# spectralcode/OCTproZ

Measured on AMD Instinct MI355X. Metric: A-scans/s, higher is better.
Workload: dtype f32

## Files before the change

octproz_amd/csrc/kernels.h:

```cpp
#pragma once
#ifndef __HIPCC_RTC__
#include <hip/hip_runtime.h>
#endif
#include <stdint.h>

#include "fft_regs.h"

namespace oct {

enum { IN_U8 = 0, IN_U16 = 1, IN_U32 = 2, IN_F32 = 3, IN_P12U = 4, IN_P12S = 5, IN_I16 = 6 };
enum { RS_NONE = 0, RS_LINEAR = 1, RS_CUBIC = 2, RS_LANCZOS = 3 };

struct FusedArgs {
	const void* raw;
	float* out;
	f2* spectrum;
	const float4* lut;
	const f2* twiddle;
	const f2* meanLine;
	unsigned numLines;
	unsigned linesInBuffer;
	unsigned ascansPerBscan;
	int bitshift;
	int rollingW;
	int rollExact;
	int flip;
	int subtractMean;
	float sA, sB;
	const float* lanczosW;
	const float* bgTerm;
	const float4* cubicW;
	float* dispBscan;
	float* dispEnFace;
	unsigned dispBscanRow0;
	unsigned dispEnFaceBin;
	unsigned dispEnFaceLast;
	const uint32_t* sinEnt;
	unsigned sinM, sinTotal, sinBlk;
};

#ifndef OCT_CW11
#define OCT_CW11 8
#endif
#ifndef OCT_PRIO_GATHER
#define OCT_PRIO_GATHER 3
#endif
#ifndef OCT_PRIO_FFT
#define OCT_PRIO_FFT 2
#endif
#ifndef OCT_PRIO_EPILOGUE
#define OCT_PRIO_EPILOGUE 1
#endif
#ifndef OCT_PRIO_STAGING
#define OCT_PRIO_STAGING 0
// ... 11 lines not shown
template <> struct GatherCfg<8> { static constexpr int GROUP = 4; static constexpr bool AHEAD = false; };
#if defined(__HIP_DEVICE_COMPILE__) && !defined(__gfx950__) && !defined(__gfx942__) && !defined(__gfx90a__)
#error "kernels.h is written for gfx9 (MI355X: gfx950)"
#endif
OCT_DEV void prologue_wait() {
	__builtin_amdgcn_s_waitcnt(0x0F70);
}
template <int LOG2N> struct Cfg;
template <> struct Cfg<8>  { static constexpr bool PLANAR = false; static constexpr int WAVES_ROLL = 0; static constexpr int WAVES = 8,  MINW = 4; static constexpr bool LDS_LUT = true; static constexpr bool PRIO = true; static constexpr bool MEAN_REGS = true; static constexpr int WAVES_CW = 8; };
template <> struct Cfg<9>  { static constexpr bool PLANAR = false; static constexpr int WAVES_ROLL = 0; static constexpr int WAVES = 8,  MINW = 4; static constexpr bool LDS_LUT = true; static constexpr bool PRIO = true; static constexpr bool MEAN_REGS = true; static constexpr int WAVES_CW = 8; };
template <> struct Cfg<10> { static constexpr bool PLANAR = false; static constexpr int WAVES_ROLL = 12; static constexpr int WAVES = 16, MINW = 4; static constexpr bool LDS_LUT = true; static constexpr bool PRIO = true; static constexpr bool MEAN_REGS = true; static constexpr int WAVES_CW = 8; };
template <> struct Cfg<11> { static constexpr bool PLANAR = true; static constexpr int WAVES_ROLL = OCT_CW11 ? 5 : 6; static constexpr int WAVES = 12, MINW = 3; static constexpr bool LDS_LUT = true; static constexpr bool PRIO = true; static constexpr bool MEAN_REGS = false; static constexpr int WAVES_CW = OCT_CW11; };
template <> struct Cfg<12> { static constexpr bool PLANAR = true; static constexpr int WAVES_ROLL = 3; static constexpr int WAVES = 6,  MINW = 2; static constexpr bool LDS_LUT = false; static constexpr bool PRIO = true; static constexpr bool MEAN_REGS = false; static constexpr int WAVES_CW = 0; };
template <int LOG2N, int RS, bool ROLL = false> struct KCfg {
	static constexpr bool CW = RS == RS_CUBIC && Cfg<LOG2N>::LDS_LUT && Cfg<LOG2N>::WAVES_CW > 0;
	static constexpr bool MEAN_REGS = Cfg<LOG2N>::MEAN_REGS || (CW && LOG2N == 11);
	static constexpr bool REGTAB = CW && LOG2N <= 10;
	static constexpr bool REGLIN = !CW && LOG2N <= 10 && (RS == RS_LINEAR || RS == RS_NONE) && !ROLL;
	static constexpr bool LZ_LDS = RS == RS_LANCZOS && LOG2N <= 10 && Cfg<LOG2N>::LDS_LUT;
	static constexpr int WAVES_PLAIN = REGLIN ? (LOG2N <= 9 ? Cfg<LOG2N>::WAVES : RS == RS_NONE ? 12 : 8) : CW ? Cfg<LOG2N>::WAVES_CW : (LZ_LDS && LOG2N == 10) ? 8 : Cfg<LOG2N>::WAVES;
	static constexpr int WAVES = (ROLL && Cfg<LOG2N>::WAVES_ROLL > 0 && Cfg<LOG2N>::WAVES_ROLL < WAVES_PLAIN) ? Cfg<LOG2N>::WAVES_ROLL : WAVES_PLAIN;
	static constexpr int MINW = ((REGTAB || REGLIN) && LOG2N <= 9) ? 4 : (REGLIN && RS == RS_NONE) ? 3 : (REGTAB || REGLIN || (LZ_LDS && LOG2N == 10)) ? 2 : (ROLL && Cfg<LOG2N>::WAVES_ROLL > 0) ? (WAVES + 3) / 4 : (CW && LOG2N == 11) ? (WAVES + 3) / 4 : Cfg<LOG2N>::MINW;
};

#ifndef OCT_LANCZOS_AHEAD
#define OCT_LANCZOS_AHEAD 2
#endif
#ifndef OCT_PADK
#define OCT_PADK 1
#endif
constexpr int ROW_OFF = 12;
// ... 416 lines not shown
		f32x4* p3 = p2 + 8 * 16;
		for (int i = tid; i < 8 * 16; i += threads) {
			const int c = i >> 4, k = i & 15;
			const f2 w0 = c ? g[(2 * c - 1) * 16 + k] : f2{1.0f, 0.0f}, w1 = g[(2 * c) * 16 + k];
			p2[i] = f32x4{w0.x, w0.y, w1.x, w1.y};
		}
		for (int i = tid; i < 6 * 64; i += threads) {
			const int c = i >> 6, l = i & 63, i0 = 2 * c, i1 = 2 * c + 1;
			const f2 w0 = g[T2 + (i0 % 3) * 256 + l + 64 * (i0 / 3)], w1 = g[T2 + (i1 % 3) * 256 + l + 64 * (i1 / 3)];
			p3[i] = f32x4{w0.x, w0.y, w1.x, w1.y};
		}
	} else {
		for (int i = tid; i < twiddle_count<LOG2N>(); i += threads) tw[i] = g[i];
	}
}
template <int LOG2N, int RS> constexpr int mean_lds_bytes() { return KCfg<LOG2N, RS>::MEAN_REGS ? 0 : (1 << LOG2N) * 4; }
template <int LOG2N, int RS, bool ROLL = false> constexpr int lut_lds_bytes() { return (!Cfg<LOG2N>::LDS_LUT || KCfg<LOG2N, RS>::REGTAB || KCfg<LOG2N, RS, ROLL>::REGLIN) ? 0 : (1 << LOG2N) * (KCfg<LOG2N, RS>::CW ? 24 : 12) + (KCfg<LOG2N, RS>::LZ_LDS ? (1 << LOG2N) * 64 : 0); }
template <int LOG2N, int RS, bool ROLL> constexpr int block_lds_bytes() {
	return tw_lds_bytes<LOG2N>() + mean_lds_bytes<LOG2N, RS>() + lut_lds_bytes<LOG2N, RS, ROLL>() + KCfg<LOG2N, RS, ROLL>::WAVES * wave_lds_bytes<(1 << LOG2N), ROLL>();
}

OCT_DEV unsigned flipped_row(const FusedArgs& a, unsigned line) {
	const unsigned b = line / a.ascansPerBscan, as = line - b * a.ascansPerBscan;
	return ((b & 1u) == 0u && (b + 2u) * a.ascansPerBscan <= a.linesInBuffer) ? b * a.ascansPerBscan + (a.ascansPerBscan - 1u - as) : line;
}
template <bool> OCT_DEV void ef_flush(const FusedArgs& a, float acc, unsigned first, unsigned stride, int lane, unsigned count) {
	if ((unsigned)lane < count) {
		const unsigned line = first + (unsigned)lane * stride;
		a.dispEnFace[a.dispEnFaceLast - (a.flip ? flipped_row(a, line) : line)] = acc;
	}
}

enum { MODE_ROLL = 1, MODE_SPECTRUM = 2, MODE_LOG = 4, MODE_BG = 8, MODE_DISP = 16, MODE_SINUS = 32 };
template <int MODE, int LOG2N, int RS> constexpr int sinus_lds_bytes() {
// ... 64 lines not shown
		const uint32_t b0 = e0.y, b1 = e0.z;
		*f0 = __builtin_bit_cast(float, b0);
		*f1 = __builtin_bit_cast(float, b1);
		const unsigned r0 = out_row();
		const bool p = sT > 0u && *f0 >= 0.0f;
		*st0 = p && r0 + 1u != lines;
		*st1 = p && *f1 >= 0.0f && r0 + 2u != lines;
		*raw = sBA0 + (e0.x & 0xffffu) + 1u == lines;
	}
};

template <int LOG2N, int INTYPE, int RS, int MODE>
__global__ __launch_bounds__((KCfg<LOG2N, RS, (MODE & 1) != 0>::WAVES) * 64, (KCfg<LOG2N, RS, (MODE & 1) != 0>::MINW)) void oct_fused_kernel(const FusedArgs a) {
	constexpr int N = 1 << LOG2N, P = N / 64;
	constexpr int WAVES = KCfg<LOG2N, RS, (MODE & MODE_ROLL) != 0>::WAVES, THREADS = WAVES * 64;
	constexpr bool LDS_LUT = Cfg<LOG2N>::LDS_LUT, CW = KCfg<LOG2N, RS>::CW, MEAN_REGS = KCfg<LOG2N, RS>::MEAN_REGS, REGTAB = KCfg<LOG2N, RS>::REGTAB;
	constexpr bool REGLIN = KCfg<LOG2N, RS, (MODE & 1) != 0>::REGLIN && RS != RS_LANCZOS;
	constexpr int RL = LastRadix<LOG2N>::value, NBL = P / RL;
	constexpr bool ROLL = (MODE & MODE_ROLL) != 0, SPECTRUM = (MODE & MODE_SPECTRUM) != 0, LOGSCALE = (MODE & MODE_LOG) != 0;
	constexpr bool SINUS = (MODE & MODE_SINUS) != 0;
	static_assert(!(SINUS && (SPECTRUM || (MODE & MODE_DISP) != 0 || RS == RS_LANCZOS)), "sinusoidal correction in the store: image output of the raw-row variants, display frames by the extraction kernel");
	typedef Chunk<INTYPE, N> CH;
	constexpr int SPL = CH::SPL, CB = CH::BYTES, NL = N / (64 * SPL);
	static_assert(!(RS == RS_LANCZOS && INTYPE != IN_F32 && INTYPE != IN_U16), "Lanczos: prepared float buffer or raw uint16 rows");
	static_assert(!(RS == RS_LANCZOS && (MODE & MODE_ROLL) != 0), "Lanczos taps cross line borders: the rolling average of the neighbour rows comes prepared");
	static_assert(!(ROLL && INTYPE != IN_U16), "in-kernel rolling average: uint16 rows only (everything else comes prepared)");
	static_assert(N / (64 * SPL) >= 1, "a row holds at least one chunk per lane");
	extern __shared__ __attribute__((aligned(16))) char smem[];
	f2* tw = reinterpret_cast<f2*>(smem);
	f2* meanL = reinterpret_cast<f2*>(smem + tw_lds_bytes<LOG2N>());
	float* rhoL = reinterpret_cast<float*>(smem + tw_lds_bytes<LOG2N>() + mean_lds_bytes<LOG2N, RS>());
	f32x4* cwL = reinterpret_cast<f32x4*>(rhoL);
	f2* wphL = reinterpret_cast<f2*>(smem + tw_lds_bytes<LOG2N>() + mean_lds_bytes<LOG2N, RS>() + N * (CW ? 16 : 4));
	constexpr bool LZ_LDS = KCfg<LOG2N, RS>::LZ_LDS;
	f32x4* lzL = reinterpret_cast<f32x4*>(smem + tw_lds_bytes<LOG2N>() + mean_lds_bytes<LOG2N, RS>() + N * 12);
	const int tid = threadIdx.x, lane = tid & 63;
	const int wave = __builtin_amdgcn_readfirstlane(tid >> 6);
	char* wbase = smem + tw_lds_bytes<LOG2N>() + mean_lds_bytes<LOG2N, RS>() + lut_lds_bytes<LOG2N, RS, ROLL>() + wave * wave_lds_bytes<N, ROLL>();
	float* row = reinterpret_cast<float*>(wbase);
	f2* xbuf = reinterpret_cast<f2*>(wbase);

	const float* termL = reinterpret_cast<const float*>(smem + block_lds_bytes<LOG2N, RS, ROLL>());
	constexpr bool SINUS_PREV_LDS = sinus_prev_lds<MODE, LOG2N, RS>();
	float* sPrevL = reinterpret_cast<float*>(smem + block_lds_bytes<LOG2N, RS, ROLL>() + bg_lds_bytes<MODE, N>()) + wave * (N / 2);
	float sPrevR[SINUS && !SINUS_PREV_LDS ? P / 2 : 1];
	if constexpr (SINUS && !SINUS_PREV_LDS) {
#pragma unroll
		for (int i = 0; i < P / 2; i++) sPrevR[i] = 0.0f;
	}
	if constexpr ((MODE & MODE_BG) != 0) fill_bg_term(reinterpret_cast<float*>(smem + block_lds_bytes<LOG2N, RS, ROLL>()), a.bgTerm, N / 2, tid, THREADS);
	fill_twiddles<LOG2N>(tw, a.twiddle, tid, THREADS);
	if constexpr (LZ_LDS) {
		const f32x4* g = reinterpret_cast<const f32x4*>(a.lanczosW);
		for (int u = tid; u < N * 4; u += THREADS) lzL[u] = g[((u & 63) + 64 * (u >> 8)) * 4 + ((u >> 6) & 3)];
	}
	if constexpr (!MEAN_REGS)
		for (int i = tid; i < N / 2; i += THREADS) meanL[i] = a.subtractMean ? a.meanLine[i] : f2{0.0f, 0.0f};
	if constexpr (LDS_LUT && !REGTAB && !REGLIN) {
		for (int i = tid; i < N; i += THREADS) {
			const float4 t = a.lut[i];
			wphL[CW ? (((i >> 7) << 6) + (i & 63)) * 2 + ((i >> 6) & 1) : i] = f2{t.y * t.z, t.y * t.w};
			if constexpr (CW) {
				const float4 w = a.cubicW[i];
				cwL[i] = f32x4{w.x, w.y, w.z, w.w};
			} else {
				rhoL[i] = t.x;
			}
		}
	}
	__syncthreads();

	const unsigned wavesTotal = gridDim.x * (unsigned)WAVES;
#ifndef OCT_DISP_BLOCK
#define OCT_DISP_BLOCK 16
#endif
	constexpr unsigned BLK = (MODE & MODE_DISP) != 0 ? (unsigned)OCT_DISP_BLOCK : 1u;
	static_assert(BLK >= 1 && BLK <= 64, "a block's en-face values live in the lanes of one register");
	const unsigned blockStride = wavesTotal * BLK;
	const unsigned blk = blockIdx.x;
	unsigned line = (blk * (unsigned)WAVES + (unsigned)wave) * BLK;
	unsigned inBlock = 0;
	SinusWalk sw;
	if constexpr (SINUS) line = sw.begin(a, blk * (unsigned)WAVES + (unsigned)wave, wavesTotal);
	auto next_line = [&](unsigned ln, unsigned pos) -> unsigned {
		if (BLK > 1u && pos + 1u < BLK) return ln + 1u;
// ... 28 lines not shown
	};
	f2 mreg[MEAN_REGS && !SPECTRUM ? P / 2 : 1];
	if constexpr (MEAN_REGS && !SPECTRUM) {
#pragma unroll
		for (int u = 0; u < RL / 2; u++)
#pragma unroll
			for (int m = 0; m < NBL; m++)
				mreg[m + u * NBL] = a.subtractMean ? a.meanLine[fft_bin<LOG2N>(lane, m, u)] : f2{0.0f, 0.0f};
	}
	float* rowl = row + ROW_OFF + lane;
	uint32_t tapA[CW ? P : 1];
	typedef __attribute__((address_space(3))) const float lds_cfloat;
	const uint32_t tapBase = __builtin_amdgcn_readfirstlane(
	    (uint32_t)(uintptr_t)(__attribute__((address_space(3))) float*)(row + ROW_OFF - 1));

	if constexpr (CW) {
#pragma unroll
		for (int q = 0; q < P; q++) tapA[q] = tapBase + 4u * (uint32_t)(int)a.lut[lane + 64 * q].x;
	}
	f32x4 cwR[REGTAB ? P : 1];
	f2 wphR[REGTAB || REGLIN ? P : 1];
	float fracR[REGLIN && RS == RS_LINEAR ? P : 1];
	uint32_t tapL[REGLIN && RS == RS_LINEAR ? P : 1];
	if constexpr (REGLIN) {
#pragma unroll
		for (int q = 0; q < P; q++) {
			const float4 t = a.lut[lane + 64 * q];
			wphR[q] = f2{t.y * t.z, t.y * t.w};
			if constexpr (RS == RS_LINEAR) {
				fracR[q] = __builtin_amdgcn_fractf(t.x);
				tapL[q] = tapBase + 4u * (uint32_t)(int)t.x + 4u;
			}
		}
	}
	constexpr bool TW3 = (REGTAB || REGLIN) && LOG2N == 10 && !ROLL && INTYPE != IN_F32;
	constexpr bool TW2 = (REGTAB || REGLIN) && LOG2N == 10 && !ROLL;
	f32x4 tw2R[TW2 ? (TW3 ? 14 : 8) : 1];
	if constexpr (REGTAB) {
#pragma unroll
		for (int q = 0; q < P; q++) {
			const float4 t = a.lut[lane + 64 * q];
			wphR[q] = f2{t.y * t.z, t.y * t.w};
			const float4 w = a.cubicW[lane + 64 * q];
			cwR[q] = f32x4{w.x, w.y, w.z, w.w};
		}
	}
	if constexpr (TW2) {
#pragma unroll
		for (int c = 0; c < 8; c++) tw2R[c] = reinterpret_cast<const f32x4*>(tw)[c * 16 + (lane & 15)];
	}
	if constexpr (TW3) {
#pragma unroll
		for (int c = 0; c < 6; c++) tw2R[8 + c] = reinterpret_cast<const f32x4*>(tw)[8 * 16 + c * 64 + lane];
	}
	float rollCnt[ROLL ? 8 : 1], rollRc[ROLL ? 8 : 1];
	if constexpr (ROLL) {
#pragma unroll
		for (int e = 0; e < 8; e++) {
			const int j = 4 * lane + (e < 4 ? 0 : 256 * (NL - 1)) + (e & 3);
			const int lo = max(0, j - a.rollingW + 1), hi = min(N - 1, j + a.rollingW);
			rollCnt[e] = (float)(hi - lo + 1);
			rollRc[e] = __fdiv_rn(1.0f, rollCnt[e]);
		}
	}
	constexpr bool DISP = (MODE & MODE_DISP) != 0;
	static_assert(!(DISP && SPECTRUM), "display frames are copies of the image");
	const unsigned efIdx = DISP ? __builtin_amdgcn_readfirstlane(a.dispEnFaceBin >> 6) : 0u, efLane = DISP ? __builtin_amdgcn_readfirstlane(a.dispEnFaceBin & 63u) : 0u;
	float efAcc = 0.0f;
	unsigned efCount = 0, efFirst = line;
	prologue_wait();
	while (line < lineEnd) {
		if constexpr (SINUS) sw.load_ahead();
		if constexpr (RS != RS_LANCZOS) {
			bool staged = false;
			if constexpr (ROLL) {
				const int W = a.rollingW;
				{
					staged = true;
					uint32_t* pfx = reinterpret_cast<uint32_t*>(row + N + 2 * ROW_OFF);
					uint32_t base = 0;
#pragma unroll
					for (int i = 0; i < NL; i++) {
						const uint4 x = chunk_to_uint(pre[i], 0, shift);
						const uint32_t tot = x.x + x.y + x.z + x.w;
						const uint32_t incl = wave_inclusive_scan(tot);
						const uint32_t p3 = base + incl, p2 = p3 - x.w, p1 = p2 - x.z, p0 = p1 - x.y;
						*reinterpret_cast<uint4*>(&pfx[ROLL_PAD + 4 * lane + 256 * i]) = uint4{p0, p1, p2, p3};
						base += (uint32_t)__builtin_amdgcn_readlane((int)incl, 63);
					}
					static_assert(ROLL_PAD == 256, "pad writes: four entries per lane");
					*reinterpret_cast<uint4*>(&pfx[4 * lane]) = uint4{0u, 0u, 0u, 0u};
					*reinterpret_cast<uint4*>(&pfx[ROLL_PAD + N + 4 * lane]) = uint4{base, base, base, base};
					wave_sync_lds();
					const uint32_t* hiP = pfx + ROLL_PAD + 4 * lane + W;
					const uint32_t* loP = pfx + ROLL_PAD + 4 * lane - W;
					const float cntIn = (float)(2 * W), rcIn = __fdiv_rn(1.0f, cntIn);
					const bool quad = (W & 3) == 0;
					const bool fast = a.rollExact == 2;
					uint32_t wsAll[NL][4];
					if (quad) {
						uint4 h4[NL], l4[NL];
#pragma unroll
						for (int i = 0; i < NL; i++) { h4[i] = *reinterpret_cast<const uint4*>(hiP + 256 * i); l4[i] = *reinterpret_cast<const uint4*>(loP + 256 * i); }
#pragma unroll
						for (int i = 0; i < NL; i++) { wsAll[i][0] = h4[i].x - l4[i].x; wsAll[i][1] = h4[i].y - l4[i].y; wsAll[i][2] = h4[i].z - l4[i].z; wsAll[i][3] = h4[i].w - l4[i].w; }
					} else {
#pragma unroll
						for (int i = 0; i < NL; i++)
#pragma unroll
							for (int c = 0; c < 4; c++) wsAll[i][c] = hiP[256 * i + c] - loP[256 * i + c];
// ... 9 lines not shown
						if (whole) {
#pragma unroll
							for (int c = 0; c < 4; c++)
								o[c] = __builtin_fmaf((float)ws[c], -rcIn, (float)xs[c]);
						} else
#pragma unroll
						for (int c = 0; c < 4; c++) {
							const float sum = (float)ws[c];
							float cnt = cntIn, rc = rcIn;
							if (i == NL - 1) { cnt = rollCnt[4 + c]; rc = rollRc[4 + c]; }
							else if (i == 0) { cnt = rollCnt[c]; rc = rollRc[c]; }
							const float q0 = sum * rc;
							const float q = __builtin_fmaf(__builtin_fmaf(-q0, cnt, sum), rc, q0);
							o[c] = (float)xs[c] - q;
						}
						*reinterpret_cast<float4*>(&row[ROW_OFF + 4 * lane + 256 * i]) = float4{o[0], o[1], o[2], o[3]};
						if constexpr (RS == RS_CUBIC) { if (i == 0 && lane == 0) row[ROW_OFF - 1] = o[1]; }
					}
				}
			}
			if (!staged) {
#pragma unroll
				for (int i = 0; i < NL; i++) {
#pragma unroll
					for (int h = 0; h < SPL / 4; h++) {
						const float4 f = chunk_to_float<INTYPE>(pre[i], h, shift);
						*reinterpret_cast<float4*>(&row[ROW_OFF + SPL * lane + 64 * SPL * i + 4 * h]) = f;
						if constexpr (RS == RS_CUBIC) { if (i == 0 && h == 0 && lane == 0) row[ROW_OFF - 1] = f.y; }
					}
				}
			}
			unsigned next;
			if constexpr (SINUS) next = sw.peek_next();
			else next = next_line(line, inBlock);
			if (next < lineEnd) {
				const __amdgpu_buffer_rsrc_t rawR = make_rsrc(reinterpret_cast<const char*>(a.raw) + (size_t)next * rowBytes, rowBytes);
#pragma unroll
				for (int i = 0; i < NL; i++) pre[i] = load_chunk<INTYPE, N>(rawR, lane * CB, i * 64 * CB);
			}
		} else {
			const long long S = (long long)a.linesInBuffer * N;
			long long off = (long long)line * N;
			if (off < 8) off = 8;
			if (off > S - 9) off = S - 9;
			if constexpr (INTYPE == IN_U16) {
				const uint16_t* g = reinterpret_cast<const uint16_t*>(a.raw) + (off - 8);
				const long long left = (S - (off - 8)) * 2;
				const __amdgpu_buffer_rsrc_t haloR = make_rsrc(g, (uint32_t)(left < (long long)(N + 16) * 2 ? left : (long long)(N + 16) * 2));
				constexpr int UNITS = (N + 16) / 8;
#pragma unroll
				for (int i = 0; i < (UNITS + 63) / 64; i++) {
					const int u = lane + 64 * i;
					if (u < UNITS) {
// ... 223 lines not shown
#pragma unroll
						for (int m = 0; m < NBL; m++) store_image<BG>(sinus_blend(pv[m], o[m], sF1), outR1, termL, lane * 4, (64 * m + u * (N / RL)) * 4);
					}
					if (sRaw) {
#pragma unroll
						for (int m = 0; m < NBL; m++) store_image<BG>(o[m], outRL, termL, lane * 4, (64 * m + u * (N / RL)) * 4);
					}
				} else
#pragma unroll
				for (int m = 0; m < NBL; m++) {
					o[m] = store_image<BG>(o[m], outR, termL, lane * 4, (64 * m + u * (N / RL)) * 4);
					if constexpr (DISP) efVec[m + u * NBL] = o[m];
				}
				if constexpr (DISP) {
					if (dispRow) {
#pragma unroll
						for (int m = 0; m < NBL; m++) buf_store32(o[m], dispR, (63 - lane) * 4, (N / 2 - 64 - 64 * m - u * (N / RL)) * 4);
					}
				}
			}
			if constexpr (DISP) {
				const float efSel = efVec[efIdx];
				const int picked = __builtin_amdgcn_readlane(__builtin_bit_cast(int, efSel), (int)efLane);
				asm volatile("s_mov_b32 m0, %2\n\ts_nop 0\n\tv_writelane_b32 %0, %1, m0" : "+v"(efAcc) : "s"(picked), "s"(__builtin_amdgcn_readfirstlane(efCount)) : "m0");
				efCount++;
				if (efCount == BLK) {
					if (a.dispEnFace) ef_flush<true>(a, efAcc, efFirst, 1u, lane, BLK);
					efCount = 0;
					efFirst = next_line(line, inBlock);
				}
			}
		}
// ... 11 lines not shown
```

octproz_amd/csrc/octpipe_api.hip:

```cpp
#include "pipe_internal.h"
#include "side_kernels.h"

namespace octimpl {
thread_local std::string g_lastError;
thread_local bool t_inCallback = false;
}
using namespace octimpl;

namespace octimpl {

struct CallbackCtx {
	octpipe* h;
	void* buffer;
	unsigned bufferNr;
	int kind;
};

void hostCallback(void* p) {
	CallbackCtx* c = static_cast<CallbackCtx*>(p);
	octpipe* h = c->h;
	struct Scope { Scope() { t_inCallback = true; } ~Scope() { t_inCallback = false; } } scope;
	if (c->kind == 0 && h->onStreaming)
		h->onStreaming(c->buffer, h->acq.bitDepth, h->acq.samplesPerLine / 2, h->acq.ascansPerBscan, h->acq.bscansPerBuffer, h->acq.buffersPerVolume, c->bufferNr, h->user);
	else if (c->kind == 1 && h->onFloatStreaming)
// ... 243 lines not shown
	}
	if (plan.sinusFused) {
		a.sinEnt = h->d_sinusEnt;
		a.sinM = h->sinusM;
		a.sinTotal = h->sinusM * (unsigned)h->B;
		a.sinBlk = h->sinusBlocksPerWave;
	}
	if (plan.dispFused) {
		a.dispBscan = wantDisp->bscan; a.dispEnFace = wantDisp->enface;
		a.dispBscanRow0 = wantDisp->bscanRow0; a.dispEnFaceBin = wantDisp->enfaceBin; a.dispEnFaceLast = wantDisp->enfaceLast;
	}
	a.out = out;
	a.spectrum = spectrumOut;
	a.lut = h->d_lut;
	a.cubicW = h->d_cubicW;
	a.twiddle = h->d_twiddle;
	a.meanLine = h->d_meanLine;
	a.numLines = lines;
	a.linesInBuffer = (unsigned)(h->A * h->B);
	a.ascansPerBscan = (unsigned)h->A;
	a.bitshift = p.bitshift;
	a.rollingW = p.rollingAverageWindowSize;
	{
		const unsigned bits = h->acq.bitDepth > 16 ? 16 : h->acq.bitDepth;
		const uint64_t maxSample = ((1ull << bits) - 1ull) >> (p.bitshift ? 4 : 0);
		const uint64_t W = p.rollingAverageWindowSize > 0 ? (uint64_t)p.rollingAverageWindowSize : 0;
		a.rollExact = W > 0 && 2ull * W * maxSample < (1ull << 24) ? 1 : 0;
		if (a.rollExact && (W & (W - 1)) == 0 && 2ull * W * maxSample < (1ull << 23)) {
			unsigned k = 0;
			while ((1ull << k) < 2ull * W) ++k;
// ... 79 lines not shown
		b.ascansPerBscan = a.ascansPerBscan;
		b.flip = a.flip;
		b.subtractMean = a.subtractMean;
		b.sA = a.sA;
		b.sB = a.sB;
		HIP_TRY(oct::launch_bluestein(h->log2n, rs, spectrum, logScale, b, h->stream));
		break;
	}
	case oct::ROUTE_KIND_REAL2:
		HIP_TRY(oct::launch_real2(rs, logScale, a, h->stream));
		break;
	case oct::ROUTE_KIND_REAL2N:
		HIP_TRY(oct::launch_real2n(h->log2n, rs, logScale, a, h->stream));
		break;
	case oct::ROUTE_KIND_FUSED:
		HIP_TRY(oct::launch_fused(h->log2n, intype, rs, roll, spectrum, logScale, a, (h->route & OCTPIPE_ROUTE_TINY_GRID) ? 2 : 0, h->stream, &h->lastGrid));
		break;
	default:
		return fail(OCTPIPE_ERR_DEVICE, "no route for this configuration");
	}
	if (!spectrum) h->lastPath = plan.path;
	if (timed) {
		if (!lt.used) {
			if (plan.launcherTimes) HIP_TRY(hipEventRecord(t.start, h->stream));
			HIP_TRY(hipEventRecord(t.stop, h->stream));
		}
		h->timed.push_back(t);
		if (h->timed.size() >= 1024) {
			size_t done = 0;
			while (done < h->timed.size() && hipEventQuery(h->timed[done].stop) == hipSuccess) {
// ... 418 lines not shown
	if (h->outStream) hipStreamSynchronize(h->outStream);
	for (auto& t : h->timed) { hipEventDestroy(t.start); hipEventDestroy(t.stop); }
	if (h->chainDone) hipEventDestroy(h->chainDone);
	for (auto e : h->destRead) if (e) hipEventDestroy(e);
	for (int i = 0; i < 2; ++i) {
		if (h->h_bufferRegistered[i]) hipHostUnregister(h->h_buffer[i]);
		if (h->d_raw[i]) hipFree(h->d_raw[i]);
		if (h->h2dDone[i]) hipEventDestroy(h->h2dDone[i]);
		if (h->slotFree[i]) hipEventDestroy(h->slotFree[i]);
	}
	for (int i = 0; i < 2; ++i) if (h->fftPlanBatch[i] && h->fftDestroy) h->fftDestroy(h->fftPlan[i]);
	if (h->d_cplx) hipFree(h->d_cplx);
	octpipe_unregister_streaming_buffers(h);
	octpipe_unregister_float_streaming_buffers(h);
	void* bufs[] = {h->d_prepared, h->d_processed, h->d_processedAlt, h->d_sinusTmp, h->d_output, h->d_lut, h->d_twiddle, h->d_meanLine,
	                h->d_postBg, h->d_bgTerm, h->d_sinusCurve, h->d_sinusEnt, h->d_spectrum, h->d_segs, h->d_dispBscan, h->d_dispEnFace, h->d_volumeView, h->d_filter, h->d_outChirp, h->d_lutPlain, h->d_twMixed, h->d_twTeam, h->d_lanczosW, h->d_twMixedN, h->d_twMixedStatic, h->d_cubicW};
	for (void* b : bufs) if (b) hipFree(b);
	release(h->sweep);
	release(h->phaseState);
	release(h->statsState);
	release(h->peakState);
	release(h->renderState);
	release(h->surfaceState);
	if (h->stream && h->ownStream && h->copyStream && h->outStream) {
		keepIdleStreams(h->device, h->stream, h->copyStream, h->outStream);
	} else {
		if (h->copyStream) hipStreamDestroy(h->copyStream);
		if (h->outStream) hipStreamDestroy(h->outStream);
		if (h->stream && h->ownStream) hipStreamDestroy(h->stream);
	}
	delete h;
// ... 392 lines not shown
```

octproz_amd/csrc/pipe_calib.hip:

```cpp
#include "pipe_internal.h"

using namespace octimpl;

namespace oct {

__global__ __launch_bounds__(256) void oct_tap_weights_kernel(const float4* lut, float4* cw, int n) {
	const int i = blockIdx.x * blockDim.x + threadIdx.x;
	if (i >= n) return;
	const double p = (double)__builtin_amdgcn_fractf(lut[i].x);
	const double w0 = 0.5 * p * ((2.0 - p) * p - 1.0), w2 = 0.5 * p * ((4.0 - 3.0 * p) * p + 1.0), w3 = 0.5 * p * p * (p - 1.0);
	cw[i] = float4{(float)w0, (float)(1.0 - w0 - w2 - w3), (float)w2, (float)w3};
}

}

namespace octimpl {

float4 lutEntry(const octpipe* h, int j, bool unitPhasor) {
	const int N = h->N;
	const OctPipeParams& p = h->params;
	float rho = p.resampling ? h->resample[j] : (float)j;
	if (!(rho >= 0.0f)) rho = 0.0f;
	if (rho > (float)(N - 3)) rho = (float)(N - 3);
	const bool disp = p.dispersionCompensation && !unitPhasor;
	float4 e;
	e.x = rho;
// ... 25 lines not shown
	for (int j = 0; j < N; ++j) {
		float4 e = lutEntry(h, j, false);
		if (h->mixed) plain[j] = e;
		if (h->bluestein) {
			const double ang = 3.14159265358979323846 * (double)(((long long)j * j) % (2LL * N)) / (double)N;
			const double cr = cos(ang), ci = sin(ang), pr = e.z, pi = e.w;
			e.z = (float)(pr * cr - pi * ci);
			e.w = (float)(pr * ci + pi * cr);
		}
		lut[j] = e;
	}
	HIP_TRY(hipMemcpyAsync(h->d_lut, lut.data(), sizeof(float4) * N, hipMemcpyHostToDevice, h->stream));
	if (!h->d_cubicW) HIP_TRY(hipMalloc((void**)&h->d_cubicW, sizeof(float4) * N));
	hipLaunchKernelGGL(oct::oct_tap_weights_kernel, dim3((N + 255) / 256), dim3(256), 0, h->stream, h->d_lut, h->d_cubicW, N);
	HIP_TRY(hipGetLastError());
	if (h->mixed) HIP_TRY(hipMemcpyAsync(h->d_lutPlain, plain.data(), sizeof(float4) * N, hipMemcpyHostToDevice, h->stream));
	if (p.resampling && p.resamplingInterpolation == OCTPIPE_INTERP_LANCZOS) {
		std::vector<float> w;
		lanczosWeights(lut, w);
		if (h->mixed) {
			std::vector<float> r(w.size());
			for (int j = 0; j < N; ++j)
				for (int c = 0; c < 4; ++c) std::memcpy(&r[(size_t)oct::mixed1664_lanczos_unit(j, c) * 4], &w[(size_t)j * 16 + (size_t)c * 4], 16);
			w.swap(r);
		}
		if (!h->d_lanczosW) HIP_TRY(hipMalloc((void**)&h->d_lanczosW, sizeof(float) * w.size()));
		HIP_TRY(hipMemcpyAsync(h->d_lanczosW, w.data(), sizeof(float) * w.size(), hipMemcpyHostToDevice, h->stream));
		HIP_TRY(hipStreamSynchronize(h->stream));
	}
	HIP_TRY(hipStreamSynchronize(h->stream));
// ... 242 lines not shown
```

octproz_amd/csrc/pipe_internal.h:

```cpp
#pragma once
#include <dlfcn.h>
#include <sys/stat.h>
#include <hip/hip_runtime.h>

#include <cmath>
#include <cstdio>
#include <cstdlib>
#include <cstring>
#include <map>
#include <mutex>
#include <string>
#include <vector>

#include "../../include/octpipe.h"
#include "../../include/octpipe_debug.h"
#include "display_kernels.h"
#include "host_luts.h"
#include "launch.h"
#include "route.h"
#include "sample_decode.h"
#include "sinus_plan.h"

namespace octimpl {

// ... 126 lines not shown
	unsigned lastPath = 0;
	bool ownStream = true;
	hipEvent_t h2dDone[2] = {nullptr, nullptr};
	hipEvent_t slotFree[2] = {nullptr, nullptr};
	bool slotUsed[2] = {false, false};
	int slot = 0;
	int lastInputSlot = -1;

	void* d_raw[2] = {nullptr, nullptr};
	float* d_prepared = nullptr;
	float* d_processed = nullptr;
	float* d_sinusTmp = nullptr;
	void* d_output = nullptr;
	float4* d_lut = nullptr;
	float4* d_cubicW = nullptr;
	f2* d_twiddle = nullptr;
	f2* d_meanLine = nullptr;
	float* d_postBg = nullptr;
	float* d_bgTerm = nullptr;
	unsigned bgVersion = 1, bgTermVersion = 0;
	float bgTermWeight = 0.0f, bgTermOffset = 0.0f;
	float* d_sinusCurve = nullptr;
	uint32_t* d_sinusEnt = nullptr;
	unsigned sinusM = 0, sinusBlocksPerWave = 0;
	f2* d_spectrum = nullptr;
	size_t spectrumLines = 0;
	float4* d_segs = nullptr;
	float* d_dispBscan = nullptr;
	float* d_dispEnFace = nullptr;
	uint64_t displaySig = 0;
// ... 121 lines not shown
```

Before: 839.9 million.

## Precompute per-lane register image of LUT and twiddles for fused kernel prologue

Adds a calibration-time kernel that packs per-lane tap weights, windowed phasors, tap offsets, fractions and radix twiddles into a lane-contiguous image. The fused kernel then loads its register tables with coalesced 128-bit buffer loads instead of gathering and recomputing from the LUT, and defers the LDS table fill until after these loads are issued. It can skip the twiddle LDS fill and barrier when everything is register-resident. It also adds a TIGHT config that moves the mean line to LDS for roll+cubic at N=512, plus asm register-pinning hints. The changes add an extra device buffer and a new required build step for log2n up to 10.

```diff
diff --git a/octproz_amd/csrc/kernels.h b/octproz_amd/csrc/kernels.h
--- a/octproz_amd/csrc/kernels.h
+++ b/octproz_amd/csrc/kernels.h
@@ -37,7 +37,14 @@
 	unsigned dispEnFaceLast;
 	const uint32_t* sinEnt;
 	unsigned sinM, sinTotal, sinBlk;
+	const float4* regImage;
 };
+
+constexpr int reg_image_wph(int log2n) { return (1 << log2n) / 64; }
+constexpr int reg_image_tap(int log2n) { return reg_image_wph(log2n) + (1 << log2n) / 128; }
+constexpr int reg_image_frac(int log2n) { return reg_image_tap(log2n) + (1 << log2n) / 256; }
+constexpr int reg_image_tw(int log2n) { return (1 << log2n) / 32; }
+constexpr int reg_image_units(int log2n) { return reg_image_tw(log2n) + (log2n == 10 ? 14 : 0); }
 
 #ifndef OCT_CW11
 #define OCT_CW11 8
@@ -79,7 +86,8 @@
 template <> struct Cfg<12> { static constexpr bool PLANAR = true; static constexpr int WAVES_ROLL = 3; static constexpr int WAVES = 6,  MINW = 2; static constexpr bool LDS_LUT = false; static constexpr bool PRIO = true; static constexpr bool MEAN_REGS = false; static constexpr int WAVES_CW = 0; };
 template <int LOG2N, int RS, bool ROLL = false> struct KCfg {
 	static constexpr bool CW = RS == RS_CUBIC && Cfg<LOG2N>::LDS_LUT && Cfg<LOG2N>::WAVES_CW > 0;
-	static constexpr bool MEAN_REGS = Cfg<LOG2N>::MEAN_REGS || (CW && LOG2N == 11);
+	static constexpr bool TIGHT = ROLL && CW && LOG2N == 9;
+	static constexpr bool MEAN_REGS = (Cfg<LOG2N>::MEAN_REGS && !TIGHT) || (CW && LOG2N == 11);
 	static constexpr bool REGTAB = CW && LOG2N <= 10;
 	static constexpr bool REGLIN = !CW && LOG2N <= 10 && (RS == RS_LINEAR || RS == RS_NONE) && !ROLL;
 	static constexpr bool LZ_LDS = RS == RS_LANCZOS && LOG2N <= 10 && Cfg<LOG2N>::LDS_LUT;
@@ -526,10 +534,10 @@
 		for (int i = tid; i < twiddle_count<LOG2N>(); i += threads) tw[i] = g[i];
 	}
 }
-template <int LOG2N, int RS> constexpr int mean_lds_bytes() { return KCfg<LOG2N, RS>::MEAN_REGS ? 0 : (1 << LOG2N) * 4; }
+template <int LOG2N, int RS, bool ROLL = false> constexpr int mean_lds_bytes() { return KCfg<LOG2N, RS, ROLL>::MEAN_REGS ? 0 : (1 << LOG2N) * 4; }
 template <int LOG2N, int RS, bool ROLL = false> constexpr int lut_lds_bytes() { return (!Cfg<LOG2N>::LDS_LUT || KCfg<LOG2N, RS>::REGTAB || KCfg<LOG2N, RS, ROLL>::REGLIN) ? 0 : (1 << LOG2N) * (KCfg<LOG2N, RS>::CW ? 24 : 12) + (KCfg<LOG2N, RS>::LZ_LDS ? (1 << LOG2N) * 64 : 0); }
 template <int LOG2N, int RS, bool ROLL> constexpr int block_lds_bytes() {
-	return tw_lds_bytes<LOG2N>() + mean_lds_bytes<LOG2N, RS>() + lut_lds_bytes<LOG2N, RS, ROLL>() + KCfg<LOG2N, RS, ROLL>::WAVES * wave_lds_bytes<(1 << LOG2N), ROLL>();
+	return tw_lds_bytes<LOG2N>() + mean_lds_bytes<LOG2N, RS, ROLL>() + lut_lds_bytes<LOG2N, RS, ROLL>() + KCfg<LOG2N, RS, ROLL>::WAVES * wave_lds_bytes<(1 << LOG2N), ROLL>();
 }
 
 OCT_DEV unsigned flipped_row(const FusedArgs& a, unsigned line) {
@@ -624,7 +632,7 @@
 __global__ __launch_bounds__((KCfg<LOG2N, RS, (MODE & 1) != 0>::WAVES) * 64, (KCfg<LOG2N, RS, (MODE & 1) != 0>::MINW)) void oct_fused_kernel(const FusedArgs a) {
 	constexpr int N = 1 << LOG2N, P = N / 64;
 	constexpr int WAVES = KCfg<LOG2N, RS, (MODE & MODE_ROLL) != 0>::WAVES, THREADS = WAVES * 64;
-	constexpr bool LDS_LUT = Cfg<LOG2N>::LDS_LUT, CW = KCfg<LOG2N, RS>::CW, MEAN_REGS = KCfg<LOG2N, RS>::MEAN_REGS, REGTAB = KCfg<LOG2N, RS>::REGTAB;
+	constexpr bool LDS_LUT = Cfg<LOG2N>::LDS_LUT, CW = KCfg<LOG2N, RS>::CW, MEAN_REGS = KCfg<LOG2N, RS, (MODE & 1) != 0>::MEAN_REGS, REGTAB = KCfg<LOG2N, RS>::REGTAB;
 	constexpr bool REGLIN = KCfg<LOG2N, RS, (MODE & 1) != 0>::REGLIN && RS != RS_LANCZOS;
 	constexpr int RL = LastRadix<LOG2N>::value, NBL = P / RL;
 	constexpr bool ROLL = (MODE & MODE_ROLL) != 0, SPECTRUM = (MODE & MODE_SPECTRUM) != 0, LOGSCALE = (MODE & MODE_LOG) != 0;
@@ -639,14 +647,14 @@
 	extern __shared__ __attribute__((aligned(16))) char smem[];
 	f2* tw = reinterpret_cast<f2*>(smem);
 	f2* meanL = reinterpret_cast<f2*>(smem + tw_lds_bytes<LOG2N>());
-	float* rhoL = reinterpret_cast<float*>(smem + tw_lds_bytes<LOG2N>() + mean_lds_bytes<LOG2N, RS>());
+	float* rhoL = reinterpret_cast<float*>(smem + tw_lds_bytes<LOG2N>() + mean_lds_bytes<LOG2N, RS, ROLL>());
 	f32x4* cwL = reinterpret_cast<f32x4*>(rhoL);
-	f2* wphL = reinterpret_cast<f2*>(smem + tw_lds_bytes<LOG2N>() + mean_lds_bytes<LOG2N, RS>() + N * (CW ? 16 : 4));
+	f2* wphL = reinterpret_cast<f2*>(smem + tw_lds_bytes<LOG2N>() + mean_lds_bytes<LOG2N, RS, ROLL>() + N * (CW ? 16 : 4));
 	constexpr bool LZ_LDS = KCfg<LOG2N, RS>::LZ_LDS;
-	f32x4* lzL = reinterpret_cast<f32x4*>(smem + tw_lds_bytes<LOG2N>() + mean_lds_bytes<LOG2N, RS>() + N * 12);
+	f32x4* lzL = reinterpret_cast<f32x4*>(smem + tw_lds_bytes<LOG2N>() + mean_lds_bytes<LOG2N, RS, ROLL>() + N * 12);
 	const int tid = threadIdx.x, lane = tid & 63;
 	const int wave = __builtin_amdgcn_readfirstlane(tid >> 6);
-	char* wbase = smem + tw_lds_bytes<LOG2N>() + mean_lds_bytes<LOG2N, RS>() + lut_lds_bytes<LOG2N, RS, ROLL>() + wave * wave_lds_bytes<N, ROLL>();
+	char* wbase = smem + tw_lds_bytes<LOG2N>() + mean_lds_bytes<LOG2N, RS, ROLL>() + lut_lds_bytes<LOG2N, RS, ROLL>() + wave * wave_lds_bytes<N, ROLL>();
 	float* row = reinterpret_cast<float*>(wbase);
 	f2* xbuf = reinterpret_cast<f2*>(wbase);
 
@@ -658,27 +666,34 @@
 #pragma unroll
 		for (int i = 0; i < P / 2; i++) sPrevR[i] = 0.0f;
 	}
-	if constexpr ((MODE & MODE_BG) != 0) fill_bg_term(reinterpret_cast<float*>(smem + block_lds_bytes<LOG2N, RS, ROLL>()), a.bgTerm, N / 2, tid, THREADS);
-	fill_twiddles<LOG2N>(tw, a.twiddle, tid, THREADS);
-	if constexpr (LZ_LDS) {
-		const f32x4* g = reinterpret_cast<const f32x4*>(a.lanczosW);
-		for (int u = tid; u < N * 4; u += THREADS) lzL[u] = g[((u & 63) + 64 * (u >> 8)) * 4 + ((u >> 6) & 3)];
-	}
-	if constexpr (!MEAN_REGS)
-		for (int i = tid; i < N / 2; i += THREADS) meanL[i] = a.subtractMean ? a.meanLine[i] : f2{0.0f, 0.0f};
-	if constexpr (LDS_LUT && !REGTAB && !REGLIN) {
-		for (int i = tid; i < N; i += THREADS) {
-			const float4 t = a.lut[i];
-			wphL[CW ? (((i >> 7) << 6) + (i & 63)) * 2 + ((i >> 6) & 1) : i] = f2{t.y * t.z, t.y * t.w};
-			if constexpr (CW) {
-				const float4 w = a.cubicW[i];
-				cwL[i] = f32x4{w.x, w.y, w.z, w.w};
-			} else {
-				rhoL[i] = t.x;
-			}
-		}
-	}
-	__syncthreads();
+	constexpr bool TW3 = (REGTAB || REGLIN) && LOG2N == 10 && !ROLL && INTYPE != IN_F32;
+	constexpr bool TW2 = (REGTAB || REGLIN) && LOG2N == 10 && !ROLL;
+	constexpr bool LDS_TABLES = !(TW2 && TW3) || (MODE & MODE_BG) != 0 || SINUS_PREV_LDS || !MEAN_REGS;
+	constexpr bool RIMG = REGTAB || REGLIN;
+	auto fill_tables = [&]() {
+		if constexpr ((MODE & MODE_BG) != 0) fill_bg_term(reinterpret_cast<float*>(smem + block_lds_bytes<LOG2N, RS, ROLL>()), a.bgTerm, N / 2, tid, THREADS);
+		if constexpr (!(TW2 && TW3)) fill_twiddles<LOG2N>(tw, a.twiddle, tid, THREADS);
+		if constexpr (LZ_LDS) {
+			const f32x4* g = reinterpret_cast<const f32x4*>(a.lanczosW);
+			for (int u = tid; u < N * 4; u += THREADS) lzL[u] = g[((u & 63) + 64 * (u >> 8)) * 4 + ((u >> 6) & 3)];
+		}
+		if constexpr (!MEAN_REGS)
+			for (int i = tid; i < N / 2; i += THREADS) meanL[i] = a.subtractMean ? a.meanLine[i] : f2{0.0f, 0.0f};
+		if constexpr (LDS_LUT && !REGTAB && !REGLIN) {
+			for (int i = tid; i < N; i += THREADS) {
+				const float4 t = a.lut[i];
+				wphL[CW ? (((i >> 7) << 6) + (i & 63)) * 2 + ((i >> 6) & 1) : i] = f2{t.y * t.z, t.y * t.w};
+				if constexpr (CW) {
+					const float4 w = a.cubicW[i];
+					cwL[i] = f32x4{w.x, w.y, w.z, w.w};
+				} else {
+					rhoL[i] = t.x;
+				}
+			}
+		}
+		if constexpr (LDS_TABLES) __syncthreads();
+	};
+	if constexpr (!RIMG) fill_tables();
 
 	const unsigned wavesTotal = gridDim.x * (unsigned)WAVES;
 #ifndef OCT_DISP_BLOCK
@@ -737,44 +752,50 @@
 	const uint32_t tapBase = __builtin_amdgcn_readfirstlane(
 	    (uint32_t)(uintptr_t)(__attribute__((address_space(3))) float*)(row + ROW_OFF - 1));
 
-	if constexpr (CW) {
+	const __amdgpu_buffer_rsrc_t imgR = make_rsrc(a.regImage, (uint32_t)reg_image_units(LOG2N) * 1024u);
+	if constexpr (CW && !RIMG) {
 #pragma unroll
 		for (int q = 0; q < P; q++) tapA[q] = tapBase + 4u * (uint32_t)(int)a.lut[lane + 64 * q].x;
 	}
 	f32x4 cwR[REGTAB ? P : 1];
-	f2 wphR[REGTAB || REGLIN ? P : 1];
+	f2 wphR[RIMG ? P : 1];
 	float fracR[REGLIN && RS == RS_LINEAR ? P : 1];
 	uint32_t tapL[REGLIN && RS == RS_LINEAR ? P : 1];
-	if constexpr (REGLIN) {
-#pragma unroll
-		for (int q = 0; q < P; q++) {
-			const float4 t = a.lut[lane + 64 * q];
-			wphR[q] = f2{t.y * t.z, t.y * t.w};
-			if constexpr (RS == RS_LINEAR) {
-				fracR[q] = __builtin_amdgcn_fractf(t.x);
-				tapL[q] = tapBase + 4u * (uint32_t)(int)t.x + 4u;
-			}
-		}
-	}
-	constexpr bool TW3 = (REGTAB || REGLIN) && LOG2N == 10 && !ROLL && INTYPE != IN_F32;
-	constexpr bool TW2 = (REGTAB || REGLIN) && LOG2N == 10 && !ROLL;
 	f32x4 tw2R[TW2 ? (TW3 ? 14 : 8) : 1];
-	if constexpr (REGTAB) {
-#pragma unroll
-		for (int q = 0; q < P; q++) {
-			const float4 t = a.lut[lane + 64 * q];
-			wphR[q] = f2{t.y * t.z, t.y * t.w};
-			const float4 w = a.cubicW[lane + 64 * q];
-			cwR[q] = f32x4{w.x, w.y, w.z, w.w};
-		}
-	}
-	if constexpr (TW2) {
-#pragma unroll
-		for (int c = 0; c < 8; c++) tw2R[c] = reinterpret_cast<const f32x4*>(tw)[c * 16 + (lane & 15)];
-	}
-	if constexpr (TW3) {
-#pragma unroll
-		for (int c = 0; c < 6; c++) tw2R[8 + c] = reinterpret_cast<const f32x4*>(tw)[8 * 16 + c * 64 + lane];
+	if constexpr (RIMG) {
+		if constexpr (REGTAB) {
+#pragma unroll
+			for (int q = 0; q < P; q++) cwR[q] = buf_load128(imgR, lane * 16, q * 1024);
+		}
+#pragma unroll
+		for (int h = 0; h < P / 2; h++) {
+			const f32x4 t = buf_load128(imgR, lane * 16, (reg_image_wph(LOG2N) + h) * 1024);
+			wphR[2 * h] = f2{t.x, t.y};
+			wphR[2 * h + 1] = f2{t.z, t.w};
+		}
+		if constexpr (REGTAB || RS == RS_LINEAR) {
+#pragma unroll
+			for (int g = 0; g < P / 4; g++) {
+				const u32x4 t = __builtin_bit_cast(u32x4, buf_load128(imgR, lane * 16, (reg_image_tap(LOG2N) + g) * 1024));
+#pragma unroll
+				for (int k = 0; k < 4; k++) {
+					if constexpr (REGTAB) tapA[4 * g + k] = tapBase + t[k];
+					else tapL[4 * g + k] = tapBase + t[k] + 4u;
+				}
+			}
+		}
+		if constexpr (REGLIN && RS == RS_LINEAR) {
+#pragma unroll
+			for (int g = 0; g < P / 4; g++) {
+				const f32x4 t = buf_load128(imgR, lane * 16, (reg_image_frac(LOG2N) + g) * 1024);
+#pragma unroll
+				for (int k = 0; k < 4; k++) fracR[4 * g + k] = t[k];
+			}
+		}
+		if constexpr (TW2) {
+#pragma unroll
+			for (int c = 0; c < (TW3 ? 14 : 8); c++) tw2R[c] = buf_load128(imgR, lane * 16, (reg_image_tw(LOG2N) + c) * 1024);
+		}
 	}
 	float rollCnt[ROLL ? 8 : 1], rollRc[ROLL ? 8 : 1];
 	if constexpr (ROLL) {
@@ -791,6 +812,7 @@
 	const unsigned efIdx = DISP ? __builtin_amdgcn_readfirstlane(a.dispEnFaceBin >> 6) : 0u, efLane = DISP ? __builtin_amdgcn_readfirstlane(a.dispEnFaceBin & 63u) : 0u;
 	float efAcc = 0.0f;
 	unsigned efCount = 0, efFirst = line;
+	if constexpr (RIMG) fill_tables();
 	prologue_wait();
 	while (line < lineEnd) {
 		if constexpr (SINUS) sw.load_ahead();
@@ -798,6 +820,8 @@
 			bool staged = false;
 			if constexpr (ROLL) {
 				const int W = a.rollingW;
+				int ln = lane;
+				if constexpr (KCfg<LOG2N, RS, ROLL>::TIGHT) asm volatile("" : "+v"(ln));
 				{
 					staged = true;
 					uint32_t* pfx = reinterpret_cast<uint32_t*>(row + N + 2 * ROW_OFF);
@@ -808,15 +832,17 @@
 						const uint32_t tot = x.x + x.y + x.z + x.w;
 						const uint32_t incl = wave_inclusive_scan(tot);
 						const uint32_t p3 = base + incl, p2 = p3 - x.w, p1 = p2 - x.z, p0 = p1 - x.y;
-						*reinterpret_cast<uint4*>(&pfx[ROLL_PAD + 4 * lane + 256 * i]) = uint4{p0, p1, p2, p3};
+						*reinterpret_cast<uint4*>(&pfx[ROLL_PAD + 4 * ln + 256 * i]) = uint4{p0, p1, p2, p3};
 						base += (uint32_t)__builtin_amdgcn_readlane((int)incl, 63);
 					}
 					static_assert(ROLL_PAD == 256, "pad writes: four entries per lane");
-					*reinterpret_cast<uint4*>(&pfx[4 * lane]) = uint4{0u, 0u, 0u, 0u};
-					*reinterpret_cast<uint4*>(&pfx[ROLL_PAD + N + 4 * lane]) = uint4{base, base, base, base};
+					uint32_t zero = 0u;
+					if constexpr (KCfg<LOG2N, RS, ROLL>::TIGHT) asm volatile("" : "+v"(zero));
+					*reinterpret_cast<uint4*>(&pfx[4 * ln]) = uint4{zero, zero, zero, zero};
+					*reinterpret_cast<uint4*>(&pfx[ROLL_PAD + N + 4 * ln]) = uint4{base, base, base, base};
 					wave_sync_lds();
-					const uint32_t* hiP = pfx + ROLL_PAD + 4 * lane + W;
-					const uint32_t* loP = pfx + ROLL_PAD + 4 * lane - W;
+					const uint32_t* hiP = pfx + ROLL_PAD + 4 * ln + W;
+					const uint32_t* loP = pfx + ROLL_PAD + 4 * ln - W;
 					const float cntIn = (float)(2 * W), rcIn = __fdiv_rn(1.0f, cntIn);
 					const bool quad = (W & 3) == 0;
 					const bool fast = a.rollExact == 2;
@@ -856,8 +882,8 @@
 							const float q = __builtin_fmaf(__builtin_fmaf(-q0, cnt, sum), rc, q0);
 							o[c] = (float)xs[c] - q;
 						}
-						*reinterpret_cast<float4*>(&row[ROW_OFF + 4 * lane + 256 * i]) = float4{o[0], o[1], o[2], o[3]};
-						if constexpr (RS == RS_CUBIC) { if (i == 0 && lane == 0) row[ROW_OFF - 1] = o[1]; }
+						*reinterpret_cast<float4*>(&row[ROW_OFF + 4 * ln + 256 * i]) = float4{o[0], o[1], o[2], o[3]};
+						if constexpr (RS == RS_CUBIC) { if (i == 0 && ln == 0) row[ROW_OFF - 1] = o[1]; }
 					}
 				}
 			}
@@ -877,8 +903,10 @@
 			else next = next_line(line, inBlock);
 			if (next < lineEnd) {
 				const __amdgpu_buffer_rsrc_t rawR = make_rsrc(reinterpret_cast<const char*>(a.raw) + (size_t)next * rowBytes, rowBytes);
-#pragma unroll
-				for (int i = 0; i < NL; i++) pre[i] = load_chunk<INTYPE, N>(rawR, lane * CB, i * 64 * CB);
+				int rowOff = lane * CB;
+				if constexpr (DISP) asm volatile("" : "+v"(rowOff));
+#pragma unroll
+				for (int i = 0; i < NL; i++) pre[i] = load_chunk<INTYPE, N>(rawR, rowOff, i * 64 * CB);
 			}
 		} else {
 			const long long S = (long long)a.linesInBuffer * N;
@@ -1132,8 +1160,10 @@
 				}
 				if constexpr (DISP) {
 					if (dispRow) {
-#pragma unroll
-						for (int m = 0; m < NBL; m++) buf_store32(o[m], dispR, (63 - lane) * 4, (N / 2 - 64 - 64 * m - u * (N / RL)) * 4);
+						int revLane = lane;
+						asm volatile("" : "+v"(revLane));
+#pragma unroll
+						for (int m = 0; m < NBL; m++) buf_store32(o[m], dispR, (63 - revLane) * 4, (N / 2 - 64 - 64 * m - u * (N / RL)) * 4);
 					}
 				}
 			}
diff --git a/octproz_amd/csrc/octpipe_api.hip b/octproz_amd/csrc/octpipe_api.hip
--- a/octproz_amd/csrc/octpipe_api.hip
+++ b/octproz_amd/csrc/octpipe_api.hip
@@ -281,6 +281,7 @@
 	a.spectrum = spectrumOut;
 	a.lut = h->d_lut;
 	a.cubicW = h->d_cubicW;
+	a.regImage = h->d_regImage;
 	a.twiddle = h->d_twiddle;
 	a.meanLine = h->d_meanLine;
 	a.numLines = lines;
@@ -390,6 +391,7 @@
 		HIP_TRY(oct::launch_real2n(h->log2n, rs, logScale, a, h->stream));
 		break;
 	case oct::ROUTE_KIND_FUSED:
+		if (h->log2n <= 10 && !a.regImage) return fail(OCTPIPE_ERR_DEVICE, "the fused kernel's register image has not been built for this handle");
 		HIP_TRY(oct::launch_fused(h->log2n, intype, rs, roll, spectrum, logScale, a, (h->route & OCTPIPE_ROUTE_TINY_GRID) ? 2 : 0, h->stream, &h->lastGrid));
 		break;
 	default:
@@ -838,7 +840,7 @@
 	octpipe_unregister_streaming_buffers(h);
 	octpipe_unregister_float_streaming_buffers(h);
 	void* bufs[] = {h->d_prepared, h->d_processed, h->d_processedAlt, h->d_sinusTmp, h->d_output, h->d_lut, h->d_twiddle, h->d_meanLine,
-	                h->d_postBg, h->d_bgTerm, h->d_sinusCurve, h->d_sinusEnt, h->d_spectrum, h->d_segs, h->d_dispBscan, h->d_dispEnFace, h->d_volumeView, h->d_filter, h->d_outChirp, h->d_lutPlain, h->d_twMixed, h->d_twTeam, h->d_lanczosW, h->d_twMixedN, h->d_twMixedStatic, h->d_cubicW};
+	                h->d_postBg, h->d_bgTerm, h->d_sinusCurve, h->d_sinusEnt, h->d_spectrum, h->d_segs, h->d_dispBscan, h->d_dispEnFace, h->d_volumeView, h->d_filter, h->d_outChirp, h->d_lutPlain, h->d_twMixed, h->d_twTeam, h->d_lanczosW, h->d_twMixedN, h->d_twMixedStatic, h->d_cubicW, h->d_regImage};
 	for (void* b : bufs) if (b) hipFree(b);
 	release(h->sweep);
 	release(h->phaseState);
diff --git a/octproz_amd/csrc/pipe_calib.hip b/octproz_amd/csrc/pipe_calib.hip
--- a/octproz_amd/csrc/pipe_calib.hip
+++ b/octproz_amd/csrc/pipe_calib.hip
@@ -10,6 +10,43 @@
 	const double p = (double)__builtin_amdgcn_fractf(lut[i].x);
 	const double w0 = 0.5 * p * ((2.0 - p) * p - 1.0), w2 = 0.5 * p * ((4.0 - 3.0 * p) * p + 1.0), w3 = 0.5 * p * p * (p - 1.0);
 	cw[i] = float4{(float)w0, (float)(1.0 - w0 - w2 - w3), (float)w2, (float)w3};
+}
+
+__global__ __launch_bounds__(256) void oct_reg_image_kernel(const float4* lut, const float4* cw, const f2* tw, int t2, float4* img, int log2n) {
+	const int i = blockIdx.x * blockDim.x + threadIdx.x;
+	if (i >= reg_image_units(log2n) * 64) return;
+	const int u = i >> 6, l = i & 63, P = (1 << log2n) / 64;
+	float4 o;
+	if (u < reg_image_wph(log2n)) {
+		o = cw[l + 64 * u];
+	} else if (u < reg_image_tap(log2n)) {
+		const int q = 2 * (u - reg_image_wph(log2n));
+		const float4 t0 = lut[l + 64 * q], t1 = lut[l + 64 * (q + 1)];
+		o = float4{t0.y * t0.z, t0.y * t0.w, t1.y * t1.z, t1.y * t1.w};
+	} else if (u < reg_image_frac(log2n)) {
+		const int q = 4 * (u - reg_image_tap(log2n));
+		uint32_t a[4];
+		for (int k = 0; k < 4; k++) a[k] = 4u * (uint32_t)(int)lut[l + 64 * (q + k)].x;
+		o = float4{__builtin_bit_cast(float, a[0]), __builtin_bit_cast(float, a[1]), __builtin_bit_cast(float, a[2]), __builtin_bit_cast(float, a[3])};
+	} else if (u < 2 * P) {
+		const int q = 4 * (u - reg_image_frac(log2n));
+		o = float4{__builtin_amdgcn_fractf(lut[l + 64 * q].x), __builtin_amdgcn_fractf(lut[l + 64 * (q + 1)].x), __builtin_amdgcn_fractf(lut[l + 64 * (q + 2)].x),
+		           __builtin_amdgcn_fractf(lut[l + 64 * (q + 3)].x)};
+	} else {
+		const int c = u - 2 * P;
+		f2 w0, w1;
+		if (c < 8) {
+			const int k = l & 15;
+			w0 = c ? tw[(2 * c - 1) * 16 + k] : f2{1.0f, 0.0f};
+			w1 = tw[(2 * c) * 16 + k];
+		} else {
+			const int i0 = 2 * (c - 8), i1 = i0 + 1;
+			w0 = tw[t2 + (i0 % 3) * 256 + l + 64 * (i0 / 3)];
+			w1 = tw[t2 + (i1 % 3) * 256 + l + 64 * (i1 / 3)];
+		}
+		o = float4{w0.x, w0.y, w1.x, w1.y};
+	}
+	img[i] = o;
 }
 
 }
@@ -65,6 +102,15 @@
 	if (!h->d_cubicW) HIP_TRY(hipMalloc((void**)&h->d_cubicW, sizeof(float4) * N));
 	hipLaunchKernelGGL(oct::oct_tap_weights_kernel, dim3((N + 255) / 256), dim3(256), 0, h->stream, h->d_lut, h->d_cubicW, N);
 	HIP_TRY(hipGetLastError());
+	if (h->d_twiddle && !h->bluestein && h->N == (1 << h->log2n) && h->log2n >= 8 && h->log2n <= 10) {
+		const int units = oct::reg_image_units(h->log2n);
+		if (!h->d_regImage) HIP_TRY(hipMalloc((void**)&h->d_regImage, sizeof(float4) * 64 * units));
+		int radices[4];
+		if (oct::fused_twiddle_plan(h->log2n, radices) < 0) return fail(OCTPIPE_ERR_UNSUPPORTED, "no FFT plan for this samplesPerLine");
+		hipLaunchKernelGGL(oct::oct_reg_image_kernel, dim3((units * 64 + 255) / 256), dim3(256), 0, h->stream, h->d_lut, h->d_cubicW, h->d_twiddle,
+		                   (radices[1] - 1) * radices[0], h->d_regImage, h->log2n);
+		HIP_TRY(hipGetLastError());
+	}
 	if (h->mixed) HIP_TRY(hipMemcpyAsync(h->d_lutPlain, plain.data(), sizeof(float4) * N, hipMemcpyHostToDevice, h->stream));
 	if (p.resampling && p.resamplingInterpolation == OCTPIPE_INTERP_LANCZOS) {
 		std::vector<float> w;
diff --git a/octproz_amd/csrc/pipe_internal.h b/octproz_amd/csrc/pipe_internal.h
--- a/octproz_amd/csrc/pipe_internal.h
+++ b/octproz_amd/csrc/pipe_internal.h
@@ -164,6 +164,7 @@
 	void* d_output = nullptr;
 	float4* d_lut = nullptr;
 	float4* d_cubicW = nullptr;
+	float4* d_regImage = nullptr;
 	f2* d_twiddle = nullptr;
 	f2* d_meanLine = nullptr;
 	float* d_postBg = nullptr;
```

After: 835.5 million. Within noise of the previous version (-0.5%).
